# reazon-research/ReazonSpeech

Measured on AMD Instinct MI355X. Metric: RTFx (audio-sec/wall-sec), FastConformer-RNNT 619M batch=256, higher is better.
Workload: dtype bf16

## Files before the change

### reazonspeech_amd/csrc/k_rnnt.hip

```cpp
#include <cstdio>
#include <cstdlib>

#include "k_rnnt_common.h"

namespace {

__global__ void rnnt_init_kernel(DecodeState st, const int32_t* __restrict__ enc_lens, int B, int blank,
                                 int32_t* __restrict__ n_ids) {
    __shared__ int n_alive_s;
    if (threadIdx.x == 0) n_alive_s = 0;
    __syncthreads();
    for (int b = threadIdx.x; b < B; b += blockDim.x) {
        st.tcur[b] = 0; st.sym[b] = 0; st.token[b] = blank; st.act[b] = b;
        if (st.token2) st.token2[b] = -1;
        n_ids[b] = 0;
        if (enc_lens[b] > 0) st.alive[atomicAdd(&n_alive_s, 1)] = b;
    }
    __syncthreads();
    if (threadIdx.x == 0) { st.counters[0] = B; st.counters[1] = 0; st.counters[2] = n_alive_s; st.counters[3] = 0; }
}

__global__ __launch_bounds__(1024) void rnnt_lstm_kernel(DecodeState st, int layer, int B, int H,
                                                        const float* __restrict__ embed,
                                                        const float* __restrict__ W ,
                                                        const float* __restrict__ bias ) {
    extern __shared__ __attribute__((aligned(16))) char lstm_smem[];
    float (*part)[4][32][16] = reinterpret_cast<float (*)[4][32][16]>(lstm_smem);
    int* rows_s = reinterpret_cast<int*>(lstm_smem + SPLITK_LSTM * 4 * 32 * 16 * 4);
    const int n_act = st.counters[0];
    const int rt = blockIdx.y, ut = blockIdx.x;
    if (rt * 32 >= n_act) return;
    const int tid = threadIdx.x, lane = tid & 63, wave = tid >> 6;
    if (tid < 32) {
        const int i = rt * 32 + tid;
        rows_s[tid] = st.act[i < n_act ? i : n_act - 1];
    }
// ... 323 lines not shown
        for (int ctile = lane; ctile < n_ctiles; ctile += 64) {
            const float ov = st.pmax[row * n_ctiles + ctile];
            const int oi = st.pidx[row * n_ctiles + ctile];
            if (ov > val || (ov == val && oi < idx)) { val = ov; idx = oi; }
        }
#pragma unroll
        for (int off = 32; off > 0; off >>= 1) {
            const float ov = __shfl_xor(val, off, 64);
            const int oi = __shfl_xor(idx, off, 64);
            if (ov > val || (ov == val && oi < idx)) { val = ov; idx = oi; }
        }
        if (idx == blank || idx == st.unk || idx == 0x7fffffff) { t += 1; sy = 0; continue; }
        if (lane == 0) {
            const int n = n_ids[b];
            if (n < u_max) { ids[(size_t)b * u_max + n] = idx; frames[(size_t)b * u_max + n] = t; n_ids[b] = n + 1; }
            else st.counters[1] = 1;
            if (st.token2) st.token2[b] = st.token[b];
            st.token[b] = idx;
        }
        emitted = true;
        sy += 1;
        if (sy >= max_symbols) { t += 1; sy = 0; }
        break;
    }
    if (lane != 0) return;
    st.tcur[b] = t; st.sym[b] = sy;
    if (t < T) {
        const int pos = atomicAdd(&st.counters[2 + ((step + 1) & 1)], 1);
        st.alive[(size_t)((step + 1) & 1) * B + pos] = b;
        if (emitted) { const int pa = atomicAdd(&st.counters[0], 1); st.act[pa] = b; }
    }
}

__global__ __launch_bounds__(1024) void rnnt_lstm4_kernel(DecodeState st, int layer, int B, int H,
                                                         const float* __restrict__ embed,
                                                         const float* __restrict__ W4 ,
                                                         const float* __restrict__ bias ) {
    __shared__ float part[SPLITK_LSTM][32][17];
    __shared__ int rows_s[32];
    const int n_act = st.counters[0];
    const int rt = blockIdx.y, ug = blockIdx.x;
    if (rt * 32 >= n_act) return;
    const int tid = threadIdx.x, lane = tid & 63, wave = tid >> 6;
    if (tid < 32) {
        const int i = rt * 32 + tid;
        rows_s[tid] = st.act[i < n_act ? i : n_act - 1];
    }
    __syncthreads();
    const int li = lane & 15, kk = lane >> 4;
    const int lr = lane >> 2, lc = lane & 3;
    const int perm = 4 * (4 * li + kk);
    const int K = 2 * H, kslice = K / SPLITK_LSTM, nkb = K / 16;
    const float* xsrc[2];
    const float* hsrc[2];
#pragma unroll
    for (int ri = 0; ri < 2; ++ri) {
        const int row = rows_s[ri * 16 + lr];
        xsrc[ri] = layer == 0 ? embed + (size_t)st.token[row] * H : st.h_tmp + ((size_t)(layer - 1) * B + row) * H;
        hsrc[ri] = st.h + ((size_t)layer * B + row) * H;
    }
    const float* wfrag = W4 + ((size_t)ug * nkb) * 256 + lane * 4;
    f32x4_t acc[2] = {(f32x4_t){0.f, 0.f, 0.f, 0.f}, (f32x4_t){0.f, 0.f, 0.f, 0.f}};
    const int kbeg = wave * kslice, nblk = kslice / 16;
    float4 av[2][8], wv[8];
#pragma unroll
    for (int u = 0; u < 8; ++u)
        if (u < nblk) {
            const int k = kbeg + 16 * u + 4 * lc;
#pragma unroll
            for (int ri = 0; ri < 2; ++ri)
                av[ri][u] = (k < H) ? *reinterpret_cast<const float4*>(xsrc[ri] + k) : *reinterpret_cast<const float4*>(hsrc[ri] + (k - H));
            wv[u] = *reinterpret_cast<const float4*>(wfrag + (size_t)((kbeg >> 4) + u) * 256);
        }
#pragma unroll
    for (int u = 0; u < 8; ++u)
        if (u < nblk) {
            const float4 a0 = to_mfma_a_layout(av[0][u], perm), a1 = to_mfma_a_layout(av[1][u], perm);
#define RS_MFMA_E(c)                                                                         \
            acc[0] = __builtin_amdgcn_mfma_f32_16x16x4f32(a0.c, wv[u].c, acc[0], 0, 0, 0);   \
            acc[1] = __builtin_amdgcn_mfma_f32_16x16x4f32(a1.c, wv[u].c, acc[1], 0, 0, 0);
            RS_MFMA_E(x) RS_MFMA_E(y) RS_MFMA_E(z) RS_MFMA_E(w)
#undef RS_MFMA_E
        }
#pragma unroll
    for (int ri = 0; ri < 2; ++ri)
#pragma unroll
        for (int r = 0; r < 4; ++r) part[wave][ri * 16 + 4 * kk + r][li] = acc[ri][r];
    __syncthreads();
    if (tid >= 128) return;
    const int i = tid >> 2, u4 = tid & 3;
    if (rt * 32 + i >= n_act) return;
    const int brow = rows_s[i];
    const int unit = ug * 4 + u4;
    float z[4];
#pragma unroll
    for (int gt = 0; gt < 4; ++gt) {
        float sm = part[0][i][gt * 4 + u4];
#pragma unroll
        for (int sl = 1; sl < SPLITK_LSTM; ++sl) sm = sm + part[sl][i][gt * 4 + u4];
        z[gt] = sm + bias[gt * H + unit];
    }
    const float ig = rs_sigmoidf(z[0]), fg = rs_sigmoidf(z[1]), gg = rs_tanhf(z[2]), og = rs_sigmoidf(z[3]);
    const size_t o = ((size_t)layer * B + brow) * H + unit;
    const float cn = fmaf(fg, st.c[o], ig * gg);
    st.c_tmp[o] = cn;
    st.h_tmp[o] = og * rs_tanhf(cn);
}

__global__ __launch_bounds__(512) void rnnt_pred16_kernel(DecodeState st, int B, int L, int H, int N ,
                                                         const float* __restrict__ W, const float* __restrict__ bias) {
    __shared__ float part[SPLITK_TILE][32][17];
    __shared__ int rows_s[32];
    const int rt = blockIdx.y, ct = blockIdx.x;
    const int tid = threadIdx.x, lane = tid & 63, wave = tid >> 6;
    const int n_rows = st.counters[0];
    if (rt * 32 >= n_rows) return;
    if (tid < 32) {
        const int i = rt * 32 + tid;
        rows_s[tid] = st.act[i < n_rows ? i : n_rows - 1];
    }
    __syncthreads();
    const int li = lane & 15, kk = lane >> 4;
    const int lr = lane >> 2, lc = lane & 3;
    const int perm = 4 * (4 * li + kk);
    const int K = H, nkb = K / 16;
    const float* asrc[2];
#pragma unroll
    for (int ri = 0; ri < 2; ++ri) asrc[ri] = st.h_tmp + ((size_t)(L - 1) * B + rows_s[ri * 16 + lr]) * H;
    const float* wfrag = W + ((size_t)ct * nkb) * 256 + lane * 4;
    f32x4_t acc[2] = {(f32x4_t){0.f, 0.f, 0.f, 0.f}, (f32x4_t){0.f, 0.f, 0.f, 0.f}};
    const int kslice = K / SPLITK_TILE, kbeg = wave * kslice, nblk = kslice / 16;
    float4 av[2][8], wv[8];
#pragma unroll
    for (int u = 0; u < 8; ++u)
        if (u < nblk) {
            const int k = kbeg + 16 * u + 4 * lc;
#pragma unroll
            for (int ri = 0; ri < 2; ++ri) av[ri][u] = *reinterpret_cast<const float4*>(asrc[ri] + k);
            wv[u] = *reinterpret_cast<const float4*>(wfrag + (size_t)((kbeg >> 4) + u) * 256);
        }
#pragma unroll
    for (int u = 0; u < 8; ++u)
        if (u < nblk) {
            const float4 a0 = to_mfma_a_layout(av[0][u], perm), a1 = to_mfma_a_layout(av[1][u], perm);
#define RS_MFMA_E(c)                                                                         \
            acc[0] = __builtin_amdgcn_mfma_f32_16x16x4f32(a0.c, wv[u].c, acc[0], 0, 0, 0);   \
            acc[1] = __builtin_amdgcn_mfma_f32_16x16x4f32(a1.c, wv[u].c, acc[1], 0, 0, 0);
            RS_MFMA_E(x) RS_MFMA_E(y) RS_MFMA_E(z) RS_MFMA_E(w)
#undef RS_MFMA_E
        }
#pragma unroll
    for (int ri = 0; ri < 2; ++ri)
#pragma unroll
        for (int r = 0; r < 4; ++r) part[wave][ri * 16 + 4 * kk + r][li] = acc[ri][r];
    __syncthreads();
    const int i = tid >> 4, c = tid & 15;
    const bool row_ok = rt * 32 + i < n_rows;
    const int brow = rows_s[i];
    const int v = ct * 16 + c;
    if (row_ok && v < N) {
        float sm = part[0][i][c];
#pragma unroll
        for (int sl = 1; sl < SPLITK_TILE; ++sl) sm = sm + part[sl][i][c];
        st.g[(size_t)brow * N + v] = sm + bias[v];
    }
    if (row_ok) {
        const int nct = gridDim.x;
        for (int l = 0; l < L; ++l)
            for (int u = ct * 16 + c; u < H; u += nct * 16) {
                const size_t o = ((size_t)l * B + brow) * H + u;
                st.h[o] = st.h_tmp[o];
                st.c[o] = st.c_tmp[o];
            }
    }
}

__global__ __launch_bounds__(256) void rnnt_prep_kernel(DecodeState st, const float* __restrict__ f, int B, int Tp, int J,
                                                        int step) {
    const int lane = threadIdx.x & 63;
    const int slot = blockIdx.x * 4 + (threadIdx.x >> 6);
    if (blockIdx.x == 0 && threadIdx.x == 0) {
        st.counters[0] = 0;
        st.counters[2 + ((step + 1) & 1)] = 0;
    }
    if (slot >= st.counters[2 + (step & 1)]) return;
    const int b = st.alive[(size_t)(step & 1) * B + slot];
    int t = st.tcur[b];
    t = t < Tp ? t : Tp - 1;
    const float* fr = f + ((size_t)b * Tp + t) * J;
    const float* gr = st.g + (size_t)b * J;
    float ss = 0.0f;
    for (int k = 4 * lane; k < J; k += 256) {
        const float4 fv = *reinterpret_cast<const float4*>(fr + k), gv = *reinterpret_cast<const float4*>(gr + k);
        float a0, a1, a2, a3;
        if (st.joint_act) {
            a0 = rs_tanhf(fv.x + gv.x); a1 = rs_tanhf(fv.y + gv.y); a2 = rs_tanhf(fv.z + gv.z); a3 = rs_tanhf(fv.w + gv.w);
        } else {
            a0 = fmaxf(fv.x + gv.x, 0.0f); a1 = fmaxf(fv.y + gv.y, 0.0f); a2 = fmaxf(fv.z + gv.z, 0.0f); a3 = fmaxf(fv.w + gv.w, 0.0f);
        }
        ss = fmaf(a0, a0, fmaf(a1, a1, fmaf(a2, a2, fmaf(a3, a3, ss))));
        *reinterpret_cast<u16x4_t*>(st.a16 + (size_t)slot * J + k) = pack_bf16x4(a0, a1, a2, a3);
    }
    ss = wave_sum(ss);
    if (lane == 0) st.anorm[slot] = sqrtf(ss) * 1.0001f;
}

// ... 257 lines not shown

namespace {

__global__ __launch_bounds__(256) void k2_decoder_kernel(DecodeState st, int B, int D, const float* __restrict__ embed,
                                                         const float* __restrict__ conv_w ) {
    const int n_rows = st.counters[0];
    if ((int)blockIdx.x >= n_rows) return;
    const int row = st.act[blockIdx.x];
    const int t0 = st.token2[row], t1 = st.token[row];
    for (int c = threadIdx.x; c < D; c += 256) {
        const int g4 = c & ~3;
        float acc = 0.0f;
#pragma unroll
        for (int i = 0; i < 4; ++i) {
            const float e = t0 >= 0 ? embed[(size_t)t0 * D + g4 + i] : 0.0f;
            acc = fmaf(conv_w[(c * 4 + i) * 2 + 0], e, acc);
        }
#pragma unroll
        for (int i = 0; i < 4; ++i) {
            const float e = t1 >= 0 ? embed[(size_t)t1 * D + g4 + i] : 0.0f;
            acc = fmaf(conv_w[(c * 4 + i) * 2 + 1], e, acc);
        }
        st.h_tmp[(size_t)row * D + c] = fmaxf(acc, 0.0f);
    }
}

constexpr int LSTM_LDS = SPLITK_LSTM * 4 * 32 * 16 * 4 + 32 * 4;
constexpr int TILE_LDS = SPLITK_TILE * 32 * 65 * 4 + 32 * 4;

bool narrow_kernels_usable(const rs_ctx* ctx) {
    const int L = ctx->d.pred_layers, H = ctx->d.pred_hidden;
    bool narrow = ctx->decode_narrow;
    for (int l = 0; l < L; ++l) narrow = narrow && ctx->lstm_w4[l] != nullptr;
    return narrow && 2 * H / SPLITK_LSTM / 16 <= 8 && H / SPLITK_TILE / 16 <= 8;
}

void launch_lstm_pred(rs_ctx* ctx, const DecodeState& st, int B, int rows_bound, bool narrow, hipStream_t s) {
    const int L = ctx->d.pred_layers, H = ctx->d.pred_hidden, J = ctx->d.joint_hidden;
    const int rts = (rows_bound + 31) / 32 > 0 ? (rows_bound + 31) / 32 : 1;
    if (ctx->k2_conv_w) {
        hipLaunchKernelGGL(k2_decoder_kernel, dim3(rows_bound > 0 ? rows_bound : 1), dim3(256), 0, s, st, B, H, ctx->embed, ctx->k2_conv_w);
        hipLaunchKernelGGL(rnnt_pred16_kernel, dim3((J + 15) / 16, rts), dim3(512), 0, s, st, B, 1, H, J, ctx->jpred_w, ctx->jpred_b);
        return;
    }
    if (narrow) {
        for (int l = 0; l < L; ++l)
            hipLaunchKernelGGL(rnnt_lstm4_kernel, dim3(H / 4, rts), dim3(1024), 0, s, st, l, B, H, ctx->embed, ctx->lstm_w4[l],
                               ctx->lstm_b[l]);
        hipLaunchKernelGGL(rnnt_pred16_kernel, dim3((J + 15) / 16, rts), dim3(512), 0, s, st, B, L, H, J, ctx->jpred_w,
                           ctx->jpred_b);
        return;
    }
    for (int l = 0; l < L; ++l)
        hipLaunchKernelGGL(rnnt_lstm_kernel, dim3(H / 16, rts), dim3(1024), LSTM_LDS, s, st, l, B, H, ctx->embed,
                           ctx->lstm_w[l], ctx->lstm_b[l]);
    hipLaunchKernelGGL(rnnt_tile_kernel<0>, dim3((J + 63) / 64, rts), dim3(512), TILE_LDS, s, st, (const float*)nullptr, B,
                       0, L, H, H, J, ctx->jpred_w, ctx->jpred_b, 0, 0, 1);
}

int joint_grid_x(int nct, int rts) {
    return rts > 1 && !rs_knob(RS_KNOB_DECODE_NO_XCD) ? (nct + 7) / 8 * 8 : nct;
}

int ensure_decode_lds(rs_ctx* ctx) {
    if (int rc = rs_ensure_dynamic_lds(ctx, (const void*)rnnt_lstm_kernel, LSTM_LDS); rc != RS_OK) return rc;
    if (int rc = rs_ensure_dynamic_lds(ctx, (const void*)rnnt_tile_kernel<0>, TILE_LDS); rc != RS_OK) return rc;
    if (int rc = rs_ensure_dynamic_lds(ctx, (const void*)rnnt_tile_kernel<1>, TILE_LDS); rc != RS_OK) return rc;
    if (int rc = rs_ensure_dynamic_lds(ctx, (const void*)rnnt_tile_kernel<2>, TILE_LDS); rc != RS_OK) return rc;
    if (int rc = rs_ensure_dynamic_lds(ctx, (const void*)rnnt_tile_kernel<3>, TILE_LDS); rc != RS_OK) return rc;
    if (int rc = rs_ensure_dynamic_lds(ctx, (const void*)rnnt_tile_kernel<4>, TILE_LDS); rc != RS_OK) return rc;
    return rs_ensure_dynamic_lds(ctx, (const void*)rnnt_tile_kernel<5>, TILE_LDS);
}

}

int rs_rnnt_launch_lstm_pred(rs_ctx* ctx, const void* st_ptr, int rows, hipStream_t s) {
    if (int rc = ensure_decode_lds(ctx); rc != RS_OK) return rc;
    launch_lstm_pred(ctx, *reinterpret_cast<const DecodeState*>(st_ptr), rows, rows, narrow_kernels_usable(ctx), s);
    return RS_OK;
}

int rs_rnnt_launch_joint_logits(rs_ctx* ctx, const void* st_ptr, const float* joint_enc, int rows, int tp_max, int rows_per_utt,
                                int step, hipStream_t s) {
    if (int rc = ensure_decode_lds(ctx); rc != RS_OK) return rc;
    const rs_dims& d = ctx->d;
    const int nct = (d.n_logits + 63) / 64;
    hipLaunchKernelGGL(rnnt_tile_kernel<2>, dim3(joint_grid_x(nct, (rows + 31) / 32), (rows + 31) / 32), dim3(512), TILE_LDS, s,
                       *reinterpret_cast<const DecodeState*>(st_ptr), joint_enc, rows, tp_max, d.pred_layers, d.pred_hidden,
                       d.joint_hidden, d.n_logits, ctx->jout_w, ctx->jout_b, nct, step, rows_per_utt);
    return RS_OK;
}

int rs_rnnt_launch_joint_logits_indirect(rs_ctx* ctx, const void* st_ptr, const float* joint_enc, int rows, int rows_bound, int tp_max,
                                         int rows_per_utt, int step, hipStream_t s) {
    if (int rc = ensure_decode_lds(ctx); rc != RS_OK) return rc;
    const rs_dims& d = ctx->d;
    const int nct = (d.n_logits + 63) / 64;
    const int rts = (rows_bound + 31) / 32 > 0 ? (rows_bound + 31) / 32 : 1;
    const DecodeState& st = *reinterpret_cast<const DecodeState*>(st_ptr);
    if (st.a_pre)
        hipLaunchKernelGGL(rnnt_tile_kernel<4>, dim3(joint_grid_x(nct, rts), rts), dim3(512), TILE_LDS, s, st, joint_enc, rows, tp_max,
                           d.pred_layers, d.pred_hidden, d.joint_hidden, d.n_logits, ctx->jout_w, ctx->jout_b, nct, step, rows_per_utt);
    else
        hipLaunchKernelGGL(rnnt_tile_kernel<3>, dim3(joint_grid_x(nct, rts), rts), dim3(512), TILE_LDS, s, st, joint_enc, rows, tp_max,
                           d.pred_layers, d.pred_hidden, d.joint_hidden, d.n_logits, ctx->jout_w, ctx->jout_b, nct, step, rows_per_utt);
    return RS_OK;
}

constexpr int LOOKAHEAD_MAX = 8;

static void greedy_layout(const rs_ctx* ctx, int B, rs_arena& a, DecodeState& st) {
// ... 12 lines not shown
    st.a16 = a.take<uint16_t>(B * J); st.anorm = a.take<float>(B);
    st.zapprox = a.take<float>(B * Vpad);
}
constexpr size_t GREEDY_SLACK = 1024;

size_t rs_rnnt_workspace_bytes(const rs_ctx* ctx, int B) {
    rs_arena a;
    DecodeState st{};
    greedy_layout(ctx, B, a, st);
    return a.bytes() + GREEDY_SLACK;
}

int rs_rnnt_greedy_impl(rs_ctx* ctx, const float* joint_enc, const int32_t* enc_lens, int B, int tp_max, int u_max,
                        int32_t* ids, int32_t* frames, int32_t* n_ids, void* workspace, size_t workspace_bytes,
                        hipStream_t s) {
    const rs_dims& d = ctx->d;
    const int L = d.pred_layers, H = d.pred_hidden, J = d.joint_hidden, V = d.n_logits;
    if (B <= 0) return RS_OK;
    if (H % 128 || J % 128) return rs_fail(ctx, RS_EINVAL, "rnnt: pred_hidden/joint_hidden must be multiples of 128");
    if (L < 1 || L > 4) return rs_fail(ctx, RS_EINVAL, "rnnt: 1..4 LSTM layers supported");
    rs_arena arena(workspace);
    DecodeState st{};
    greedy_layout(ctx, B, arena, st);
    if (workspace_bytes < arena.bytes() + GREEDY_SLACK) return rs_fail(ctx, RS_EWORKSPACE, "rnnt: workspace too small");
    st.joint_act = d.joint_act;
    if (ctx->k2_conv_w) st.unk = ctx->k2 ? rs_k2_unk_id(ctx) : -1;
    const size_t state_bytes = (size_t)L * B * H * 4;
    const int nct = (V + 63) / 64, Vpad = (V + 15) / 16 * 16;
    const bool screen = ctx->decode_screen && ctx->jout_w16 && ctx->jout_wrm && ctx->jout_bpad && ctx->jout_wmax &&
                        J / SPLITK_TILE / 16 <= 8 && J / 32 <= 20;

    if (int rc = ensure_decode_lds(ctx); rc != RS_OK) return rc;
    const bool narrow = narrow_kernels_usable(ctx);
    auto lstm_and_pred = [&](int rows_bound) { launch_lstm_pred(ctx, st, B, rows_bound, narrow, s); };

    rs_prof_begin(ctx, RS_PROF_DECODE, s, 0.0, 0.0);
    RS_HIP(ctx, hipMemsetAsync(st.h, 0, 2 * rs_align(state_bytes), s));
    RS_HIP(ctx, hipMemsetAsync(st.g, 0, (size_t)B * J * 4, s));
    hipLaunchKernelGGL(rnnt_init_kernel, dim3(1), dim3(256), 0, s, st, enc_lens, B, d.blank_id, n_ids);
    lstm_and_pred(B);
    RS_CHECK_LAUNCH(ctx, "rnnt init");

    const int max_steps = tp_max + (u_max < tp_max * d.max_symbols ? u_max : tp_max * d.max_symbols) + 1;
    const int CHUNK = 16;
    const bool lookahead = !rs_knob(RS_KNOB_DECODE_NO_LOOKAHEAD);
    const bool verify_wide = rs_knob(RS_KNOB_VERIFY_WIDE) != 0;
    int32_t host_counters[4] = {0, 0, 0, 0};
    int steps = 0, alive_bound = B;
    bool finished = false;
    while (!finished && steps < max_steps) {
        for (int c = 0; c < CHUNK; ++c, ++steps) {
            const int rows = alive_bound < B ? alive_bound : B;
            if (screen) {
                const int rts = (rows + 31) / 32 > 0 ? (rows + 31) / 32 : 1;
                hipLaunchKernelGGL(rnnt_prep_kernel, dim3((rows + 3) / 4 > 0 ? (rows + 3) / 4 : 1), dim3(256), 0, s, st, joint_enc, B,
                                   tp_max, J, steps);
                hipLaunchKernelGGL(rnnt_screen_kernel, dim3((Vpad + 63) / 64, rts), dim3(256), 32 * (J * 2 + 16), s, st, joint_enc, B,
                                   tp_max, J, Vpad, ctx->jout_w16, ctx->jout_bpad, steps);
                const dim3 vg((rows + 3) / 4 > 0 ? (rows + 3) / 4 : 1), vgw(rows > 0 ? rows : 1);
#define RS_VERIFY_ARGS st, joint_enc, enc_lens, B, tp_max, J, V, Vpad, ctx->jout_wrm, ctx->jout_b, ctx->jout_wmax, d.blank_id, d.max_symbols, u_max, steps, ids, frames, n_ids
                if (V > 64 * 48 && V <= 4 * 64 * 48)
                    hipLaunchKernelGGL(rnnt_verify_wide_kernel<48>, vgw, dim3(256), J * 4 + 4 * 48 * 64 * 4 + 64, s, RS_VERIFY_ARGS);
                else if (V > 64 * 48)
                    hipLaunchKernelGGL(rnnt_verify_kernel<0>, vg, dim3(256), 4 * J * 4 + 4 * VER_CAP * 4, s, RS_VERIFY_ARGS);
                else if (verify_wide)
                    hipLaunchKernelGGL(rnnt_verify_wide_kernel<12>, vgw, dim3(256), J * 4 + 4 * 12 * 64 * 4 + 64, s, RS_VERIFY_ARGS);
                else if (V <= 64 * 8)
                    hipLaunchKernelGGL(rnnt_verify_kernel<8>, vg, dim3(256), 4 * J * 4 + 4 * 8 * 64 * 4, s, RS_VERIFY_ARGS);
                else
                    hipLaunchKernelGGL(rnnt_verify_kernel<48>, vg, dim3(256), 4 * J * 4 + 4 * 48 * 64 * 4, s, RS_VERIFY_ARGS);
#undef RS_VERIFY_ARGS
            } else {
                int la = 1;
                if (lookahead) while (la < LOOKAHEAD_MAX && 2 * la * (rows > 0 ? rows : 1) <= 256) la *= 2;
                if (la > 1) {
                    const int rts = (rows * la + 31) / 32 > 0 ? (rows * la + 31) / 32 : 1;
                    hipLaunchKernelGGL(rnnt_tile_kernel<5>, dim3(joint_grid_x(nct, rts), rts), dim3(512), TILE_LDS, s, st, joint_enc, B, tp_max, L, H,
                                       J, V, ctx->jout_w, ctx->jout_b, nct, steps, la);
                    hipLaunchKernelGGL(rnnt_finalize_la_kernel, dim3((rows + 3) / 4 > 0 ? (rows + 3) / 4 : 1), dim3(256), 0, s, st, enc_lens, B, nct,
                                       d.blank_id, d.max_symbols, u_max, steps, la, ids, frames, n_ids);
                } else {
                    const int rts = (rows + 31) / 32 > 0 ? (rows + 31) / 32 : 1;
                    hipLaunchKernelGGL(rnnt_tile_kernel<1>, dim3(joint_grid_x(nct, rts), rts), dim3(512), TILE_LDS, s, st, joint_enc, B, tp_max, L, H,
                                       J, V, ctx->jout_w, ctx->jout_b, nct, steps, 1);
                    hipLaunchKernelGGL(rnnt_finalize_kernel, dim3((rows + 3) / 4 > 0 ? (rows + 3) / 4 : 1), dim3(256), 0, s, st, enc_lens, B, nct,
                                       d.blank_id, d.max_symbols, u_max, steps, ids, frames, n_ids);
                }
            }
            lstm_and_pred(rows);
        }
        RS_CHECK_LAUNCH(ctx, "rnnt step");
        RS_HIP(ctx, hipMemcpyAsync(host_counters, st.counters, 4 * sizeof(int32_t), hipMemcpyDeviceToHost, s));
        RS_HIP(ctx, hipStreamSynchronize(s));
        finished = host_counters[2 + (steps & 1)] == 0;
        alive_bound = host_counters[2 + (steps & 1)];
    }
    rs_prof_end(ctx, RS_PROF_DECODE, s);
    if (rs_knob(RS_KNOB_DECODE_TRACE)) fprintf(stderr, "[decode trace] B=%d T'=%d: %d steps (screen %d, narrow %d, lookahead %d)\n", B, tp_max, steps, (int)screen, (int)narrow, (int)lookahead);
    if (host_counters[1]) return rs_fail(ctx, RS_EOVERFLOW, "rnnt: an utterance emitted more than u_max=%d tokens", u_max);
    if (!finished) return rs_fail(ctx, RS_ESTATE, "rnnt: decode did not finish in %d steps", max_steps);
    return RS_OK;
}
```

### reazonspeech_amd/csrc/rs_api.hip

```cpp
#include <stdarg.h>
#include <stdlib.h>
#include <string.h>

#include <mutex>
#include <set>
#include <utility>

#include "rs_common.h"

size_t rs_rnnt_workspace_bytes(const rs_ctx* ctx, int B);
size_t rs_rnnt_alsd_workspace_bytes_impl(const rs_ctx* ctx, int B, int beam, int cap);
size_t rs_rnnt_mbs_workspace_bytes_impl(const rs_ctx* ctx, int B, int K, int tp_max);
int rs_rnnt_mbs_impl(rs_ctx* ctx, const float* joint_enc, const int32_t* enc_lens, int B, int tp_max, int K, float blank_penalty,
                     int length_norm, int out_cap, int32_t* ids, int32_t* frames, int32_t* n_ids, float* scores, void* workspace,
                     size_t workspace_bytes, hipStream_t s);
size_t rs_rnnt_beam_workspace_bytes_impl(const rs_ctx* ctx, int B, int beam, int tp_max, int max_pops);
int rs_rnnt_beam_impl(rs_ctx* ctx, const float* joint_enc, const int32_t* enc_lens, int B, int tp_max, int beam, int score_norm,
                      int max_pops, int out_cap, int32_t* ids, int32_t* frames, int32_t* n_ids, float* scores, int32_t* pops,
                      void* workspace, size_t workspace_bytes, hipStream_t s);
int rs_rnnt_alsd_impl(rs_ctx* ctx, const float* joint_enc, const int32_t* enc_lens, int B, int tp_max, int beam, double ratio,
                      int abs_len, int score_norm, int merge, int out_cap, int32_t* ids, int32_t* steps, int32_t* n_ids,
                      float* scores, void* workspace, size_t workspace_bytes, hipStream_t s);
size_t rs_ctc_align_workspace_bytes_impl(int B, int tp_max, int c_max);
int rs_ctc_align_impl(rs_ctx* ctx, const float* probs, int ld, const int32_t* enc_lens, int B, int tp_max, const int32_t* gt,
// ... 80 lines not shown
    if (!out || !dims) return RS_EINVAL;
    *out = nullptr;
    rs_ctx* ctx = new (std::nothrow) rs_ctx();
    if (!ctx) return RS_EINVAL;
    ctx->device = device;
    ctx->d = *dims;
    const rs_dims& d = ctx->d;
    int rc = RS_OK;
    if (d.n_heads <= 0 || d.d_model % d.n_heads || (d.d_model / d.n_heads != 128 && d.d_model / d.n_heads != 64))
        rc = rs_fail(ctx, RS_EINVAL, "head_dim must be 128 or 64 (d_model %d, heads %d)", d.d_model, d.n_heads);
    else if (d.d_model % 256 || d.ff_dim % 64) rc = rs_fail(ctx, RS_EINVAL, "d_model %% 256, ff_dim %% 64 required");
    else if (d.sub_stages < 2 || d.sub_stages > 4) rc = rs_fail(ctx, RS_EINVAL, "2..4 subsampling stages supported");
    else if (d.n_layers < 1) rc = rs_fail(ctx, RS_EINVAL, "n_layers");
    else if (d.pred_layers < 1 || d.pred_layers > 4) rc = rs_fail(ctx, RS_EINVAL, "pred_layers");
    else if ((unsigned)d.frontend_kind > 1u  || (unsigned)d.sub_kind > 1u || (unsigned)d.final_norm > 1u || (unsigned)d.joint_act > 1u)
        rc = rs_fail(ctx, RS_EINVAL, "model family switches must be 0 or 1");
    else if (d.sub_kind == 1 && (d.sub_stages != 2 || d.sub_channels % 64)) rc = rs_fail(ctx, RS_EINVAL, "Conv2dSubsampling: x4 (two stages), channels %% 64");
    else if (d.frontend_kind == 1 && d.preemph != 0.0f) rc = rs_fail(ctx, RS_EINVAL, "the ESPnet front-end has no pre-emphasis");
    else if (d.ctc_vocab < 0) rc = rs_fail(ctx, RS_EINVAL, "ctc_vocab < 0");
    if (rc != RS_OK) { *out = ctx; return rc; }
    ctx->head_dim = d.d_model / d.n_heads;
    int f = d.n_mels;
    for (int s = 0; s < d.sub_stages; ++s) f = rs_conv_len(f, d.sub_kind);
    ctx->sub_freq = f;
    if (hipSetDevice(device) != hipSuccess) { *out = ctx; return rs_fail(ctx, RS_EHIP, "hipSetDevice(%d) failed", device); }
    *out = ctx;
    return RS_OK;
}

void rs_destroy(rs_ctx* ctx) {
    if (!ctx) return;
    for (auto& p : ctx->prof)
        for (auto e : p.ev) hipEventDestroy(e);
    for (auto& kv : ctx->wfm) (void)hipFree(kv.second);
    if (ctx->wfm_scratch) (void)hipFree(ctx->wfm_scratch);
    if (ctx->k2 && ctx->k2_free) ctx->k2_free(ctx->k2);
    if (ctx->avsr && ctx->avsr_free) ctx->avsr_free(ctx->avsr);
    delete ctx;
}

const char* rs_last_error(const rs_ctx* ctx) { return ctx ? ctx->err.c_str() : "null context"; }

int rs_set_tensor(rs_ctx* ctx, const char* name, const void* dev_ptr, size_t nbytes) {
    if (!ctx || !name || !dev_ptr) return RS_EINVAL;
    ctx->tensors[name] = {dev_ptr, nbytes};
    ctx->finalized = false;
    return RS_OK;
}

}

namespace {

struct Resolver {
    rs_ctx* ctx;
    int rc = RS_OK;
    template <typename T>
    void get(const std::string& name, size_t elems, const T*& out) {
        if (rc != RS_OK) return;
        auto it = ctx->tensors.find(name);
        if (it == ctx->tensors.end()) { rc = rs_fail(ctx, RS_EMISSING, "weight tensor '%s' was not registered", name.c_str()); return; }
        if (it->second.second != elems * sizeof(T)) {
            rc = rs_fail(ctx, RS_EINVAL, "tensor '%s': expected %zu bytes, got %zu", name.c_str(), elems * sizeof(T),
                         it->second.second);
            return;
        }
// ... 729 lines not shown
```

### reazonspeech_amd/csrc/rs_common.h

```cpp
#pragma once
#include <hip/hip_runtime.h>
#include <stdint.h>
#include <stdio.h>
#include <string>
#include <unordered_map>
#include <vector>

#include "../../include/rs_asr.h"
#include "rs_arena.h"
#include "rs_knobs.h"

typedef __bf16 bf16x8_t __attribute__((ext_vector_type(8)));
typedef float f32x4_t __attribute__((ext_vector_type(4)));
typedef float f32x16_t __attribute__((ext_vector_type(16)));
typedef unsigned short u16x8_t __attribute__((ext_vector_type(8)));
typedef unsigned short u16x4_t __attribute__((ext_vector_type(4)));

__device__ __forceinline__ float bf16_to_f32(unsigned short v) {
    return __uint_as_float(((unsigned)v) << 16);
}
typedef __bf16 bf16x4_t __attribute__((ext_vector_type(4)));
typedef __bf16 bf16x2_t __attribute__((ext_vector_type(2)));
__device__ __forceinline__ unsigned short f32_to_bf16(float f) {
    return __builtin_bit_cast(unsigned short, (__bf16)f);
// ... 86 lines not shown
    const float* sub_conv1_b = nullptr;
    const float *final_norm_g = nullptr, *final_norm_b = nullptr;
    const uint16_t* ctc_w = nullptr;
    const float* ctc_b = nullptr;
    float *ctc_probs = nullptr, *ctc_blank = nullptr;
    const uint16_t* jenc_w = nullptr;
    const float* jenc_b = nullptr;
    const float* lstm_w4[8] = {};
    const float* k2_conv_w = nullptr;
    const float *embed = nullptr, *lstm_w[8] = {}, *lstm_b[8] = {}, *jpred_w = nullptr, *jpred_b = nullptr,
                *jout_w = nullptr, *jout_b = nullptr;
    const uint16_t* jout_w16 = nullptr;
    const float *jout_wrm = nullptr, *jout_bpad = nullptr, *jout_wmax = nullptr;
    bool decode_screen = true;
    bool decode_narrow = true;
    bool gemm_f32_x3 = false;
    int k2_conv2_fused = -1;
    int k2_cnx_fused = -1;
    int n_cus = 0;
    int defer_out_norm = 1;
    int fuse_glu = 1;
    bool has_f32 = false;
    int precision_f32 = 0;
    bool has_i8 = false;
    int precision_i8 = 0;
    rs_f32_weights f32;
    bool env_read = false;
    float* tap_sub = nullptr;
    float* tap_layers = nullptr;
    std::vector<int> tap_ids;
    std::unordered_map<const void*, void*> wfm;
    void* wfm_scratch = nullptr;
    size_t wfm_scratch_bytes = 0;
    int prof_mask = 0;
    rs_prof_slot prof[8];
    int32_t prof_tag[4] = {0, 0, 0, 0};
};

int rs_ensure_dynamic_lds(rs_ctx* ctx, const void* func, int bytes);

int rs_fail(rs_ctx* ctx, int code, const char* fmt, ...);
int rs_n_cus(rs_ctx* ctx);

#define RS_HIP(ctx, call)                                                              \
    do {                                                                               \
        hipError_t _e = (call);                                                        \
        if (_e != hipSuccess)                                                          \
            return rs_fail((ctx), RS_EHIP, "%s:%d %s -> %s", __FILE__, __LINE__, #call, \
                           hipGetErrorString(_e));                                     \
    } while (0)

#define RS_CHECK_LAUNCH(ctx, what)                                                            \
    do {                                                                                      \
        hipError_t _e = hipGetLastError();                                                    \
        if (_e != hipSuccess)                                                                 \
            return rs_fail((ctx), RS_EHIP, "launch %s failed: %s", (what), hipGetErrorString(_e)); \
    } while (0)

int rs_prof_class_index(int klass);
void rs_prof_begin(rs_ctx* ctx, int klass, hipStream_t s, double flops, double bytes);
void rs_prof_end(rs_ctx* ctx, int klass, hipStream_t s);

struct rs_gemm_args {
    const uint16_t* A; int lda;
    const uint16_t* W; int ldw;
    void* out; int ldc;
// ... 62 lines not shown
```

### reazonspeech_amd/csrc/rs_knobs.h

```cpp
#pragma once
#include <stdlib.h>
#include <string.h>

#include <atomic>
#include <mutex>

#include "../../include/rs_asr.h"

#define RS_KNOBS(X)                                                                                                                   \
    X(GEMM_TILE, "RS_GEMM_TILE", INT, 0, "forced GEMM tile height (256 / 192 / 128 / 64); 0 = by shape")                              \
    X(GEMM_GROUP_M, "RS_GEMM_GROUP_M", INT, 0, "row panels per XCD tile group; 0 = by shape")                                         \
    X(GEMM_PAIRS, "RS_GEMM_PAIRS", INT, 2, "2 = two tiles per workgroup, LDS ring carried over; 1 = ring restarted; 0 = one tile")    \
    X(GEMM_BREG, "RS_GEMM_BREG", INT, 0, "1 = 256- / 192-row launches keep the weight operand out of LDS (global -> VGPR)")           \
    X(ATTN_PERSIST, "RS_ATTN_PERSIST", INT, 0, "1 = full attention on resident workgroups that walk the items (n >= 2: on n)")        \
    X(ATTN_STREAM, "RS_ATTN_STREAM", INT, 0, "1 = the streaming attention form (+ 16 x mask: phases left out, for timing)")           \
    X(ATTN64, "RS_ATTN64", INT, 4, "head_dim 64: key blocks per chunk; 0 = the one-workgroup-per-CU geometry")                        \
    X(ATTN64_NW, "RS_ATTN64_NW", INT, 4, "head_dim 64: waves per workgroup (the second number of $RS_ATTN64)")                        \
    X(ATTN_F32_OLD, "RS_ATTN_F32_OLD", PRESENT, 0, "float32 attention: the first form (one wave per key sum)")                        \
    X(ATTN_F32_KEYS, "RS_ATTN_F32_KEYS", PRESENT, 0, "float32 attention: the second form (keys over lanes, no MFMA)")                 \
    X(GLU_GENERIC, "RS_GLU_GENERIC", INT, 0, "GLU + depthwise conv: 1 = the any-kernel-size path, 2 = the f32-tile kernel on the gated layout") \
    X(SUB_IM2COL, "RS_SUB_IM2COL", PRESENT, 0, "ESPnet subsampling: gather the 3 x 3 patches into a matrix first (sizes the workspace too)") \
    X(FUSE_GLU, "RS_FUSE_GLU", INT, 1, "context default: 0 = GLU in the depthwise kernel, not the pw1 GEMM epilogue")                 \
    X(DEFER_OUT_NORM, "RS_DEFER_OUT_NORM", INT, 1, "context default: 0 = every output norm stores its f32 rows")                      \
    X(DECODE_SCREEN, "RS_DECODE_SCREEN", INT, 1, "context default: 0 = exact evaluation of every joint column")                       \
    X(DECODE_NARROW, "RS_DECODE_NARROW", INT, 1, "context default: 0 = the wide-tile LSTM / projection kernels")                      \
    X(DECODE_NO_XCD, "RS_DECODE_NO_XCD", PRESENT, 0, "greedy decode: joint grids not padded to a multiple of 8 column tiles")         \
    X(DECODE_NO_LOOKAHEAD, "RS_DECODE_NO_LOOKAHEAD", PRESENT, 0, "greedy decode: one frame per utterance and step at every batch size") \
    X(VERIFY_WIDE, "RS_VERIFY_WIDE", INT, 0, "screened joint: 1 = a workgroup per row for V <= 3072 too")                             \
    X(DECODE_TRACE, "RS_DECODE_TRACE", PRESENT, 0, "greedy decode: print the step count of every call to stderr")                     \
    X(BEAM_SPEC, "RS_BEAM_SPEC", INT, 3, "beam search: evaluations asked for per iteration (1 .. 8; sizes the workspace too)")         \
    X(BEAM_TRACE, "RS_BEAM_TRACE", PRESENT, 0, "beam search: phase timing of the step kernel")                                        \
    X(BEAM_RECORD_LDS, "RS_BEAM_RECORD_LDS", PRESENT, 0, "beam search: the any-vocabulary record kernel on a small vocabulary")       \
    X(AVSR_POSCONV_OLD, "RS_AVSR_POSCONV_OLD", PRESENT, 0, "AV-HuBERT positional convolution: the VALU form")                         \
    X(K2_CONV1_OLD, "RS_K2_CONV1_OLD", PRESENT, 0, "Zipformer conv1: the VALU form (the one other channel counts run)")               \
    X(K2_ATTW_SWEEPS, "RS_K2_ATTW_SWEEPS", INT, 1, "Zipformer attention weights: 3 = the three-sweep kernel")                         \
    X(K2_CONV2_FUSED, "RS_K2_CONV2_FUSED", INT, 1, "default of option k2_conv2_fused: 0 = patch matrix + GEMM launch")                \
    X(K2_CNX_FUSED, "RS_K2_CNX_FUSED", INT, 1, "default of option k2_cnx_fused: 0 = the ConvNeXt pointwise pair as two GEMM launches")

enum rs_knob_id {
#define RS_KNOB_ENUM(id, env, kind, def, what) RS_KNOB_##id,
    RS_KNOBS(RS_KNOB_ENUM)
#undef RS_KNOB_ENUM
    RS_KNOB_COUNT
};
enum rs_knob_kind { RS_KNOB_PRESENT, RS_KNOB_INT };
struct rs_knob_row { const char* env; rs_knob_kind kind; int def; };
static const rs_knob_row rs_knob_rows[RS_KNOB_COUNT] = {
#define RS_KNOB_ROW(id, env, kind, def, what) {env, RS_KNOB_##kind, def},
    RS_KNOBS(RS_KNOB_ROW)
#undef RS_KNOB_ROW
};

struct rs_knob_table {
    std::atomic<int> value[RS_KNOB_COUNT];
    std::atomic<bool> given[RS_KNOB_COUNT];
    std::once_flag once;
};
inline rs_knob_table rs_knob_state;
// ... 40 lines not shown
```

Before: 44180.

## Pipeline greedy-decode chunk polling and template narrow LSTM kernels on block count

The greedy decode loop now copies the alive counters into pinned host memory and records an event per chunk instead of synchronizing the stream after every chunk. The host only waits on the previous chunk's event, so the next chunk is enqueued while the GPU is still running, using an alive-row bound that is one chunk stale. The narrow LSTM and projection kernels are templated on the per-wave block count and can loop over row tiles, keeping weight fragments in registers; an optional knob caps row tiles per launch (off by default). The stale bound can launch extra empty steps past completion, and the per-launch switch adds template instantiations.

Result: no change. 44450, median of 6 (+0.6%).

```diff
diff --git a/reazonspeech_amd/csrc/k_rnnt.hip b/reazonspeech_amd/csrc/k_rnnt.hip
--- a/reazonspeech_amd/csrc/k_rnnt.hip
+++ b/reazonspeech_amd/csrc/k_rnnt.hip
@@ -2,6 +2,7 @@
 #include <cstdlib>
 
 #include "k_rnnt_common.h"
+#include "rs_decode_chunks.h"
 
 namespace {
 
@@ -391,146 +392,151 @@
     }
 }
 
+template <int NBLK>
 __global__ __launch_bounds__(1024) void rnnt_lstm4_kernel(DecodeState st, int layer, int B, int H,
                                                          const float* __restrict__ embed,
                                                          const float* __restrict__ W4 ,
                                                          const float* __restrict__ bias ) {
     __shared__ float part[SPLITK_LSTM][32][17];
     __shared__ int rows_s[32];
-    const int n_act = st.counters[0];
-    const int rt = blockIdx.y, ug = blockIdx.x;
-    if (rt * 32 >= n_act) return;
+    const int n_act = __builtin_amdgcn_readfirstlane(st.counters[0]);
+    const int ug = blockIdx.x;
+    if ((int)blockIdx.y * 32 >= n_act) return;
     const int tid = threadIdx.x, lane = tid & 63, wave = tid >> 6;
-    if (tid < 32) {
-        const int i = rt * 32 + tid;
-        rows_s[tid] = st.act[i < n_act ? i : n_act - 1];
-    }
-    __syncthreads();
     const int li = lane & 15, kk = lane >> 4;
     const int lr = lane >> 2, lc = lane & 3;
     const int perm = 4 * (4 * li + kk);
     const int K = 2 * H, kslice = K / SPLITK_LSTM, nkb = K / 16;
-    const float* xsrc[2];
-    const float* hsrc[2];
-#pragma unroll
-    for (int ri = 0; ri < 2; ++ri) {
-        const int row = rows_s[ri * 16 + lr];
-        xsrc[ri] = layer == 0 ? embed + (size_t)st.token[row] * H : st.h_tmp + ((size_t)(layer - 1) * B + row) * H;
-        hsrc[ri] = st.h + ((size_t)layer * B + row) * H;
-    }
     const float* wfrag = W4 + ((size_t)ug * nkb) * 256 + lane * 4;
-    f32x4_t acc[2] = {(f32x4_t){0.f, 0.f, 0.f, 0.f}, (f32x4_t){0.f, 0.f, 0.f, 0.f}};
-    const int kbeg = wave * kslice, nblk = kslice / 16;
-    float4 av[2][8], wv[8];
-#pragma unroll
-    for (int u = 0; u < 8; ++u)
-        if (u < nblk) {
-            const int k = kbeg + 16 * u + 4 * lc;
-#pragma unroll
-            for (int ri = 0; ri < 2; ++ri)
-                av[ri][u] = (k < H) ? *reinterpret_cast<const float4*>(xsrc[ri] + k) : *reinterpret_cast<const float4*>(hsrc[ri] + (k - H));
-            wv[u] = *reinterpret_cast<const float4*>(wfrag + (size_t)((kbeg >> 4) + u) * 256);
-        }
-#pragma unroll
-    for (int u = 0; u < 8; ++u)
-        if (u < nblk) {
+    const int kbeg = wave * kslice;
+    float4 wv[NBLK];
+#pragma unroll
+    for (int u = 0; u < NBLK; ++u) wv[u] = *reinterpret_cast<const float4*>(wfrag + (size_t)((kbeg >> 4) + u) * 256);
+#pragma nounroll
+    for (int rt = blockIdx.y; rt * 32 < n_act; rt += gridDim.y) {
+        if (tid < 32) {
+            const int i = rt * 32 + tid;
+            rows_s[tid] = st.act[i < n_act ? i : n_act - 1];
+        }
+        __syncthreads();
+        const float* asrc[2];
+#pragma unroll
+        for (int ri = 0; ri < 2; ++ri) {
+            const int row = rows_s[ri * 16 + lr];
+            const float* x = layer == 0 ? embed + (size_t)st.token[row] * H : st.h_tmp + ((size_t)(layer - 1) * B + row) * H;
+            const float* h = st.h + ((size_t)layer * B + row) * H;
+            asrc[ri] = (kbeg < H ? x + kbeg : h + (kbeg - H)) + 4 * lc;
+        }
+        f32x4_t acc[2] = {(f32x4_t){0.f, 0.f, 0.f, 0.f}, (f32x4_t){0.f, 0.f, 0.f, 0.f}};
+        float4 av[2][NBLK];
+#pragma unroll
+        for (int u = 0; u < NBLK; ++u)
+#pragma unroll
+            for (int ri = 0; ri < 2; ++ri) av[ri][u] = *reinterpret_cast<const float4*>(asrc[ri] + 16 * u);
+#pragma unroll
+        for (int u = 0; u < NBLK; ++u) {
             const float4 a0 = to_mfma_a_layout(av[0][u], perm), a1 = to_mfma_a_layout(av[1][u], perm);
-#define RS_MFMA_E(c)                                                                         \
-            acc[0] = __builtin_amdgcn_mfma_f32_16x16x4f32(a0.c, wv[u].c, acc[0], 0, 0, 0);   \
+#define RS_MFMA_E(c)                                                                             \
+            acc[0] = __builtin_amdgcn_mfma_f32_16x16x4f32(a0.c, wv[u].c, acc[0], 0, 0, 0);       \
             acc[1] = __builtin_amdgcn_mfma_f32_16x16x4f32(a1.c, wv[u].c, acc[1], 0, 0, 0);
             RS_MFMA_E(x) RS_MFMA_E(y) RS_MFMA_E(z) RS_MFMA_E(w)
 #undef RS_MFMA_E
         }
 #pragma unroll
-    for (int ri = 0; ri < 2; ++ri)
-#pragma unroll
-        for (int r = 0; r < 4; ++r) part[wave][ri * 16 + 4 * kk + r][li] = acc[ri][r];
-    __syncthreads();
-    if (tid >= 128) return;
-    const int i = tid >> 2, u4 = tid & 3;
-    if (rt * 32 + i >= n_act) return;
-    const int brow = rows_s[i];
-    const int unit = ug * 4 + u4;
-    float z[4];
-#pragma unroll
-    for (int gt = 0; gt < 4; ++gt) {
-        float sm = part[0][i][gt * 4 + u4];
-#pragma unroll
-        for (int sl = 1; sl < SPLITK_LSTM; ++sl) sm = sm + part[sl][i][gt * 4 + u4];
-        z[gt] = sm + bias[gt * H + unit];
-    }
-    const float ig = rs_sigmoidf(z[0]), fg = rs_sigmoidf(z[1]), gg = rs_tanhf(z[2]), og = rs_sigmoidf(z[3]);
-    const size_t o = ((size_t)layer * B + brow) * H + unit;
-    const float cn = fmaf(fg, st.c[o], ig * gg);
-    st.c_tmp[o] = cn;
-    st.h_tmp[o] = og * rs_tanhf(cn);
-}
-
+        for (int ri = 0; ri < 2; ++ri)
+#pragma unroll
+            for (int r = 0; r < 4; ++r) part[wave][ri * 16 + 4 * kk + r][li] = acc[ri][r];
+        __syncthreads();
+        const int i = tid >> 2, u4 = tid & 3;
+        if (tid < 128 && rt * 32 + i < n_act) {
+            const int brow = rows_s[i];
+            const int unit = ug * 4 + u4;
+            float z[4];
+#pragma unroll
+            for (int gt = 0; gt < 4; ++gt) {
+                float sm = part[0][i][gt * 4 + u4];
+#pragma unroll
+                for (int sl = 1; sl < SPLITK_LSTM; ++sl) sm = sm + part[sl][i][gt * 4 + u4];
+                z[gt] = sm + bias[gt * H + unit];
+            }
+            const float ig = rs_sigmoidf(z[0]), fg = rs_sigmoidf(z[1]), gg = rs_tanhf(z[2]), og = rs_sigmoidf(z[3]);
+            const size_t o = ((size_t)layer * B + brow) * H + unit;
+            const float cn = fmaf(fg, st.c[o], ig * gg);
+            st.c_tmp[o] = cn;
+            st.h_tmp[o] = og * rs_tanhf(cn);
+        }
+        __syncthreads();
+    }
+}
+
+template <int NBLK>
 __global__ __launch_bounds__(512) void rnnt_pred16_kernel(DecodeState st, int B, int L, int H, int N ,
                                                          const float* __restrict__ W, const float* __restrict__ bias) {
     __shared__ float part[SPLITK_TILE][32][17];
     __shared__ int rows_s[32];
-    const int rt = blockIdx.y, ct = blockIdx.x;
+    const int ct = blockIdx.x;
     const int tid = threadIdx.x, lane = tid & 63, wave = tid >> 6;
-    const int n_rows = st.counters[0];
-    if (rt * 32 >= n_rows) return;
-    if (tid < 32) {
-        const int i = rt * 32 + tid;
-        rows_s[tid] = st.act[i < n_rows ? i : n_rows - 1];
-    }
-    __syncthreads();
+    const int n_rows = __builtin_amdgcn_readfirstlane(st.counters[0]);
+    if ((int)blockIdx.y * 32 >= n_rows) return;
     const int li = lane & 15, kk = lane >> 4;
     const int lr = lane >> 2, lc = lane & 3;
     const int perm = 4 * (4 * li + kk);
     const int K = H, nkb = K / 16;
-    const float* asrc[2];
-#pragma unroll
-    for (int ri = 0; ri < 2; ++ri) asrc[ri] = st.h_tmp + ((size_t)(L - 1) * B + rows_s[ri * 16 + lr]) * H;
     const float* wfrag = W + ((size_t)ct * nkb) * 256 + lane * 4;
-    f32x4_t acc[2] = {(f32x4_t){0.f, 0.f, 0.f, 0.f}, (f32x4_t){0.f, 0.f, 0.f, 0.f}};
-    const int kslice = K / SPLITK_TILE, kbeg = wave * kslice, nblk = kslice / 16;
-    float4 av[2][8], wv[8];
-#pragma unroll
-    for (int u = 0; u < 8; ++u)
-        if (u < nblk) {
-            const int k = kbeg + 16 * u + 4 * lc;
-#pragma unroll
-            for (int ri = 0; ri < 2; ++ri) av[ri][u] = *reinterpret_cast<const float4*>(asrc[ri] + k);
-            wv[u] = *reinterpret_cast<const float4*>(wfrag + (size_t)((kbeg >> 4) + u) * 256);
-        }
-#pragma unroll
-    for (int u = 0; u < 8; ++u)
-        if (u < nblk) {
+    const int kslice = K / SPLITK_TILE, kbeg = wave * kslice;
+    float4 wv[NBLK];
+#pragma unroll
+    for (int u = 0; u < NBLK; ++u) wv[u] = *reinterpret_cast<const float4*>(wfrag + (size_t)((kbeg >> 4) + u) * 256);
+#pragma nounroll
+    for (int rt = blockIdx.y; rt * 32 < n_rows; rt += gridDim.y) {
+        if (tid < 32) {
+            const int i = rt * 32 + tid;
+            rows_s[tid] = st.act[i < n_rows ? i : n_rows - 1];
+        }
+        __syncthreads();
+        const float* asrc[2];
+#pragma unroll
+        for (int ri = 0; ri < 2; ++ri) asrc[ri] = st.h_tmp + ((size_t)(L - 1) * B + rows_s[ri * 16 + lr]) * H;
+        f32x4_t acc[2] = {(f32x4_t){0.f, 0.f, 0.f, 0.f}, (f32x4_t){0.f, 0.f, 0.f, 0.f}};
+        float4 av[2][NBLK];
+#pragma unroll
+        for (int u = 0; u < NBLK; ++u)
+#pragma unroll
+            for (int ri = 0; ri < 2; ++ri) av[ri][u] = *reinterpret_cast<const float4*>(asrc[ri] + kbeg + 16 * u + 4 * lc);
+#pragma unroll
+        for (int u = 0; u < NBLK; ++u) {
             const float4 a0 = to_mfma_a_layout(av[0][u], perm), a1 = to_mfma_a_layout(av[1][u], perm);
-#define RS_MFMA_E(c)                                                                         \
-            acc[0] = __builtin_amdgcn_mfma_f32_16x16x4f32(a0.c, wv[u].c, acc[0], 0, 0, 0);   \
+#define RS_MFMA_E(c)                                                                             \
+            acc[0] = __builtin_amdgcn_mfma_f32_16x16x4f32(a0.c, wv[u].c, acc[0], 0, 0, 0);       \
             acc[1] = __builtin_amdgcn_mfma_f32_16x16x4f32(a1.c, wv[u].c, acc[1], 0, 0, 0);
             RS_MFMA_E(x) RS_MFMA_E(y) RS_MFMA_E(z) RS_MFMA_E(w)
 #undef RS_MFMA_E
         }
 #pragma unroll
-    for (int ri = 0; ri < 2; ++ri)
-#pragma unroll
-        for (int r = 0; r < 4; ++r) part[wave][ri * 16 + 4 * kk + r][li] = acc[ri][r];
-    __syncthreads();
-    const int i = tid >> 4, c = tid & 15;
-    const bool row_ok = rt * 32 + i < n_rows;
-    const int brow = rows_s[i];
-    const int v = ct * 16 + c;
-    if (row_ok && v < N) {
-        float sm = part[0][i][c];
-#pragma unroll
-        for (int sl = 1; sl < SPLITK_TILE; ++sl) sm = sm + part[sl][i][c];
-        st.g[(size_t)brow * N + v] = sm + bias[v];
-    }
-    if (row_ok) {
-        const int nct = gridDim.x;
-        for (int l = 0; l < L; ++l)
-            for (int u = ct * 16 + c; u < H; u += nct * 16) {
-                const size_t o = ((size_t)l * B + brow) * H + u;
-                st.h[o] = st.h_tmp[o];
-                st.c[o] = st.c_tmp[o];
-            }
+        for (int ri = 0; ri < 2; ++ri)
+#pragma unroll
+            for (int r = 0; r < 4; ++r) part[wave][ri * 16 + 4 * kk + r][li] = acc[ri][r];
+        __syncthreads();
+        const int i = tid >> 4, c = tid & 15;
+        const bool row_ok = rt * 32 + i < n_rows;
+        const int brow = rows_s[i];
+        const int v = ct * 16 + c;
+        if (row_ok && v < N) {
+            float sm = part[0][i][c];
+#pragma unroll
+            for (int sl = 1; sl < SPLITK_TILE; ++sl) sm = sm + part[sl][i][c];
+            st.g[(size_t)brow * N + v] = sm + bias[v];
+        }
+        if (row_ok) {
+            const int nct = gridDim.x;
+            for (int l = 0; l < L; ++l)
+                for (int u = ct * 16 + c; u < H; u += nct * 16) {
+                    const size_t o = ((size_t)l * B + brow) * H + u;
+                    st.h[o] = st.h_tmp[o];
+                    st.c[o] = st.c_tmp[o];
+                }
+        }
+        __syncthreads();
     }
 }
 
@@ -854,29 +860,40 @@
     const int L = ctx->d.pred_layers, H = ctx->d.pred_hidden;
     bool narrow = ctx->decode_narrow;
     for (int l = 0; l < L; ++l) narrow = narrow && ctx->lstm_w4[l] != nullptr;
-    return narrow && 2 * H / SPLITK_LSTM / 16 <= 8 && H / SPLITK_TILE / 16 <= 8;
-}
-
-void launch_lstm_pred(rs_ctx* ctx, const DecodeState& st, int B, int rows_bound, bool narrow, hipStream_t s) {
+    return narrow && H % 128 == 0 && H / 128 <= 8;
+}
+
+#define RS_NARROW_NBLK(n, LAUNCH)                                                                                      \
+    switch (n) {                                                                                                       \
+        case 1: LAUNCH(1); break; case 2: LAUNCH(2); break; case 3: LAUNCH(3); break; case 4: LAUNCH(4); break;        \
+        case 5: LAUNCH(5); break; case 6: LAUNCH(6); break; case 7: LAUNCH(7); break; default: LAUNCH(8); break;       \
+    }
+
+void launch_lstm_pred(rs_ctx* ctx, const DecodeState& st, int B, int rows_bound, bool narrow, int rt_cap, hipStream_t s) {
     const int L = ctx->d.pred_layers, H = ctx->d.pred_hidden, J = ctx->d.joint_hidden;
-    const int rts = (rows_bound + 31) / 32 > 0 ? (rows_bound + 31) / 32 : 1;
+    const int rts_all = (rows_bound + 31) / 32 > 0 ? (rows_bound + 31) / 32 : 1;
+    int rts = rts_all;
+    if (rt_cap > 0 && rt_cap < rts) rts = rt_cap;
     if (ctx->k2_conv_w) {
         hipLaunchKernelGGL(k2_decoder_kernel, dim3(rows_bound > 0 ? rows_bound : 1), dim3(256), 0, s, st, B, H, ctx->embed, ctx->k2_conv_w);
-        hipLaunchKernelGGL(rnnt_pred16_kernel, dim3((J + 15) / 16, rts), dim3(512), 0, s, st, B, 1, H, J, ctx->jpred_w, ctx->jpred_b);
+#define RS_PRED16(n) hipLaunchKernelGGL(rnnt_pred16_kernel<n>, dim3((J + 15) / 16, rts), dim3(512), 0, s, st, B, layers, H, J, ctx->jpred_w, ctx->jpred_b)
+        const int layers = 1;
+        RS_NARROW_NBLK(H / 128, RS_PRED16)
         return;
     }
     if (narrow) {
-        for (int l = 0; l < L; ++l)
-            hipLaunchKernelGGL(rnnt_lstm4_kernel, dim3(H / 4, rts), dim3(1024), 0, s, st, l, B, H, ctx->embed, ctx->lstm_w4[l],
-                               ctx->lstm_b[l]);
-        hipLaunchKernelGGL(rnnt_pred16_kernel, dim3((J + 15) / 16, rts), dim3(512), 0, s, st, B, L, H, J, ctx->jpred_w,
-                           ctx->jpred_b);
+#define RS_LSTM4(n) hipLaunchKernelGGL(rnnt_lstm4_kernel<n>, dim3(H / 4, rts), dim3(1024), 0, s, st, l, B, H, ctx->embed, ctx->lstm_w4[l], ctx->lstm_b[l])
+        for (int l = 0; l < L; ++l) RS_NARROW_NBLK(H / 128, RS_LSTM4)
+        const int layers = L;
+        RS_NARROW_NBLK(H / 128, RS_PRED16)
+#undef RS_LSTM4
+#undef RS_PRED16
         return;
     }
     for (int l = 0; l < L; ++l)
-        hipLaunchKernelGGL(rnnt_lstm_kernel, dim3(H / 16, rts), dim3(1024), LSTM_LDS, s, st, l, B, H, ctx->embed,
+        hipLaunchKernelGGL(rnnt_lstm_kernel, dim3(H / 16, rts_all), dim3(1024), LSTM_LDS, s, st, l, B, H, ctx->embed,
                            ctx->lstm_w[l], ctx->lstm_b[l]);
-    hipLaunchKernelGGL(rnnt_tile_kernel<0>, dim3((J + 63) / 64, rts), dim3(512), TILE_LDS, s, st, (const float*)nullptr, B,
+    hipLaunchKernelGGL(rnnt_tile_kernel<0>, dim3((J + 63) / 64, rts_all), dim3(512), TILE_LDS, s, st, (const float*)nullptr, B,
                        0, L, H, H, J, ctx->jpred_w, ctx->jpred_b, 0, 0, 1);
 }
 
@@ -898,7 +915,7 @@
 
 int rs_rnnt_launch_lstm_pred(rs_ctx* ctx, const void* st_ptr, int rows, hipStream_t s) {
     if (int rc = ensure_decode_lds(ctx); rc != RS_OK) return rc;
-    launch_lstm_pred(ctx, *reinterpret_cast<const DecodeState*>(st_ptr), rows, rows, narrow_kernels_usable(ctx), s);
+    launch_lstm_pred(ctx, *reinterpret_cast<const DecodeState*>(st_ptr), rows, rows, narrow_kernels_usable(ctx), 0, s);
     return RS_OK;
 }
 
@@ -977,7 +994,8 @@
 
     if (int rc = ensure_decode_lds(ctx); rc != RS_OK) return rc;
     const bool narrow = narrow_kernels_usable(ctx);
-    auto lstm_and_pred = [&](int rows_bound) { launch_lstm_pred(ctx, st, B, rows_bound, narrow, s); };
+    const int rt_cap = rs_knob(RS_KNOB_DECODE_ROWLOOP);
+    auto lstm_and_pred = [&](int rows_bound) { launch_lstm_pred(ctx, st, B, rows_bound, narrow, rt_cap, s); };
 
     rs_prof_begin(ctx, RS_PROF_DECODE, s, 0.0, 0.0);
     RS_HIP(ctx, hipMemsetAsync(st.h, 0, 2 * rs_align(state_bytes), s));
@@ -990,12 +1008,22 @@
     const int CHUNK = 16;
     const bool lookahead = !rs_knob(RS_KNOB_DECODE_NO_LOOKAHEAD);
     const bool verify_wide = rs_knob(RS_KNOB_VERIFY_WIDE) != 0;
-    int32_t host_counters[4] = {0, 0, 0, 0};
-    int steps = 0, alive_bound = B;
-    bool finished = false;
-    while (!finished && steps < max_steps) {
-        for (int c = 0; c < CHUNK; ++c, ++steps) {
-            const int rows = alive_bound < B ? alive_bound : B;
+    if (!ctx->decode_words) {
+        RS_HIP(ctx, hipHostMalloc(reinterpret_cast<void**>(&ctx->decode_words), 2 * 4 * sizeof(int32_t), hipHostMallocDefault));
+        for (int i = 0; i < 2; ++i) RS_HIP(ctx, hipEventCreateWithFlags(&ctx->decode_ev[i], hipEventDisableTiming));
+    }
+    rs_decode_chunks ch(B, max_steps, CHUNK, false);
+    auto look = [&](bool last) -> int {
+        for (int w; (w = ch.wait_for(last)) >= 0;) {
+            RS_HIP(ctx, hipEventSynchronize(ctx->decode_ev[w & 1]));
+            ch.look(ctx->decode_words + 4 * (w & 1));
+        }
+        return RS_OK;
+    };
+    while (ch.more()) {
+        const int rows = ch.rows();
+        for (int c = 0; c < CHUNK; ++c) {
+            const int steps = ch.steps + c;
             if (screen) {
                 const int rts = (rows + 31) / 32 > 0 ? (rows + 31) / 32 : 1;
                 hipLaunchKernelGGL(rnnt_prep_kernel, dim3((rows + 3) / 4 > 0 ? (rows + 3) / 4 : 1), dim3(256), 0, s, st, joint_enc, B,
@@ -1035,14 +1063,16 @@
             lstm_and_pred(rows);
         }
         RS_CHECK_LAUNCH(ctx, "rnnt step");
-        RS_HIP(ctx, hipMemcpyAsync(host_counters, st.counters, 4 * sizeof(int32_t), hipMemcpyDeviceToHost, s));
-        RS_HIP(ctx, hipStreamSynchronize(s));
-        finished = host_counters[2 + (steps & 1)] == 0;
-        alive_bound = host_counters[2 + (steps & 1)];
-    }
+        RS_HIP(ctx, hipMemcpyAsync(ctx->decode_words + 4 * ch.slot(), st.counters, 4 * sizeof(int32_t), hipMemcpyDeviceToHost, s));
+        RS_HIP(ctx, hipEventRecord(ctx->decode_ev[ch.slot()], s));
+        ch.enqueued();
+        if (int rc = look(false); rc != RS_OK) return rc;
+    }
+    if (int rc = look(true); rc != RS_OK) return rc;
+    RS_HIP(ctx, hipStreamSynchronize(s));
     rs_prof_end(ctx, RS_PROF_DECODE, s);
-    if (rs_knob(RS_KNOB_DECODE_TRACE)) fprintf(stderr, "[decode trace] B=%d T'=%d: %d steps (screen %d, narrow %d, lookahead %d)\n", B, tp_max, steps, (int)screen, (int)narrow, (int)lookahead);
-    if (host_counters[1]) return rs_fail(ctx, RS_EOVERFLOW, "rnnt: an utterance emitted more than u_max=%d tokens", u_max);
-    if (!finished) return rs_fail(ctx, RS_ESTATE, "rnnt: decode did not finish in %d steps", max_steps);
+    if (rs_knob(RS_KNOB_DECODE_TRACE)) fprintf(stderr, "[decode trace] B=%d T'=%d: %d steps enqueued (screen %d, narrow %d, lookahead %d)\n", B, tp_max, ch.steps, (int)screen, (int)narrow, (int)lookahead);
+    if (ch.overflow()) return rs_fail(ctx, RS_EOVERFLOW, "rnnt: an utterance emitted more than u_max=%d tokens", u_max);
+    if (!ch.finished()) return rs_fail(ctx, RS_ESTATE, "rnnt: decode did not finish in %d steps", max_steps);
     return RS_OK;
 }
diff --git a/reazonspeech_amd/csrc/rs_api.hip b/reazonspeech_amd/csrc/rs_api.hip
--- a/reazonspeech_amd/csrc/rs_api.hip
+++ b/reazonspeech_amd/csrc/rs_api.hip
@@ -136,6 +136,10 @@
     if (!ctx) return;
     for (auto& p : ctx->prof)
         for (auto e : p.ev) hipEventDestroy(e);
+    if (ctx->decode_words) {
+        (void)hipHostFree(ctx->decode_words);
+        for (auto e : ctx->decode_ev) (void)hipEventDestroy(e);
+    }
     for (auto& kv : ctx->wfm) (void)hipFree(kv.second);
     if (ctx->wfm_scratch) (void)hipFree(ctx->wfm_scratch);
     if (ctx->k2 && ctx->k2_free) ctx->k2_free(ctx->k2);
diff --git a/reazonspeech_amd/csrc/rs_common.h b/reazonspeech_amd/csrc/rs_common.h
--- a/reazonspeech_amd/csrc/rs_common.h
+++ b/reazonspeech_amd/csrc/rs_common.h
@@ -142,6 +142,8 @@
     std::unordered_map<const void*, void*> wfm;
     void* wfm_scratch = nullptr;
     size_t wfm_scratch_bytes = 0;
+    int32_t* decode_words = nullptr;
+    hipEvent_t decode_ev[2] = {};
     int prof_mask = 0;
     rs_prof_slot prof[8];
     int32_t prof_tag[4] = {0, 0, 0, 0};
diff --git a/reazonspeech_amd/csrc/rs_decode_chunks.h b/reazonspeech_amd/csrc/rs_decode_chunks.h
--- /dev/null
+++ b/reazonspeech_amd/csrc/rs_decode_chunks.h
@@ -0,0 +1,30 @@
+#pragma once
+#include <stdint.h>
+
+struct rs_decode_chunks {
+    int B, max_steps, chunk;
+    bool drain;
+    int steps = 0;
+    int queued = 0;
+    int seen = 0;
+    int alive_bound;
+    bool done = false, over = false;
+
+    rs_decode_chunks(int B_, int max_steps_, int chunk_, bool drain_)
+        : B(B_), max_steps(max_steps_), chunk(chunk_), drain(drain_), alive_bound(B_) {}
+
+    bool more() const { return !done && steps < max_steps; }
+    int rows() const { return alive_bound < B ? alive_bound : B; }
+    int slot() const { return queued & 1; }
+    void enqueued() { steps += chunk; ++queued; }
+    int wait_for(bool last) const { return seen < queued - ((last || drain) ? 0 : 1) ? seen : -1; }
+    void look(const int32_t counters[4]) {
+        const int next_step = (seen + 1) * chunk;
+        alive_bound = counters[2 + (next_step & 1)];
+        if (alive_bound == 0) done = true;
+        if (counters[1]) over = true;
+        ++seen;
+    }
+    bool finished() const { return done; }
+    bool overflow() const { return over; }
+};
diff --git a/reazonspeech_amd/csrc/rs_knobs.h b/reazonspeech_amd/csrc/rs_knobs.h
--- a/reazonspeech_amd/csrc/rs_knobs.h
+++ b/reazonspeech_amd/csrc/rs_knobs.h
@@ -24,6 +24,7 @@
     X(DEFER_OUT_NORM, "RS_DEFER_OUT_NORM", INT, 1, "context default: 0 = every output norm stores its f32 rows")                      \
     X(DECODE_SCREEN, "RS_DECODE_SCREEN", INT, 1, "context default: 0 = exact evaluation of every joint column")                       \
     X(DECODE_NARROW, "RS_DECODE_NARROW", INT, 1, "context default: 0 = the wide-tile LSTM / projection kernels")                      \
+    X(DECODE_ROWLOOP, "RS_DECODE_ROWLOOP", INT, 0, "greedy decode: n > 0 = at most n row tiles per launch of the narrow LSTM / projection kernels, the rest walked") \
     X(DECODE_NO_XCD, "RS_DECODE_NO_XCD", PRESENT, 0, "greedy decode: joint grids not padded to a multiple of 8 column tiles")         \
     X(DECODE_NO_LOOKAHEAD, "RS_DECODE_NO_LOOKAHEAD", PRESENT, 0, "greedy decode: one frame per utterance and step at every batch size") \
     X(VERIFY_WIDE, "RS_VERIFY_WIDE", INT, 0, "screened joint: 1 = a workgroup per row for V <= 3072 too")                             \
```
